# Feuermagier/Beyond_Deep_Ensembles

Hardware: NVIDIA B200
Metric: svgd_posterior_update_algorithmic_GBps (higher is better)
Workload: dtype f32

## Files before the change

beyond_deep_ensembles_b200/csrc/common.cuh:

```cuda
#pragma once
#include <cuda.h>
#include <cuda_runtime.h>
#include <cstdint>
#include <cstddef>

#include "bde_b200.h"

namespace bde {

#define BDE_RETURN_IF_CUDA(expr)                       \
    do {                                               \
        cudaError_t _e = (expr);                       \
        if (_e != cudaSuccess) return static_cast<int>(_e); \
    } while (0)

#define BDE_CHECK_LAUNCH()                             \
    do {                                               \
        cudaError_t _e = cudaGetLastError();           \
        if (_e != cudaSuccess) return static_cast<int>(_e); \
    } while (0)

inline int sm_count_cached() {
    static int cached[64] = {0};
    int dev = 0;
    if (cudaGetDevice(&dev) != cudaSuccess || dev < 0 || dev >= 64) return 148;
    if (cached[dev] == 0) {
        int v = 0;
        if (cudaDeviceGetAttribute(&v, cudaDevAttrMultiProcessorCount, dev) != cudaSuccess || v <= 0) v = 148;
        cached[dev] = v;
    }
    return cached[dev];
}

struct Tuning {
    int pairdist_ctas_per_sm = 0;
    int apply_ctas_per_sm = 0;
    int ew_ctas_per_sm = 0;
    int apply_variant = 0;
    int pairdist_variant = 0;
    int ew_variant = 0;
    int apply_tile_sets = 0;
    int swag_batch = 0;
    int batch_splits = 0;
    int batch_prefetch = 0;
    int gram_pairing = 0;
    int gram_fold = 0;
    int gram_l2_promotion = 0;
    int ring_kb = 0;
    int gram_guard_x1000 = 0;
};
Tuning& tuning();

inline bool aligned16(const void* p) { return (reinterpret_cast<uintptr_t>(p) & 15u) == 0; }

typedef unsigned long long f32x2;

__device__ __forceinline__ f32x2 pack2(float lo, float hi) {
    f32x2 r;
    asm("mov.b64 %0, {%1, %2};" : "=l"(r) : "f"(lo), "f"(hi));
    return r;
}
__device__ __forceinline__ void unpack2(f32x2 v, float& lo, float& hi) {
    asm("mov.b64 {%0, %1}, %2;" : "=f"(lo), "=f"(hi) : "l"(v));
}
__device__ __forceinline__ f32x2 sub2(f32x2 a, f32x2 b) {
    f32x2 r;
    asm("sub.f32x2 %0, %1, %2;" : "=l"(r) : "l"(a), "l"(b));
    return r;
}
__device__ __forceinline__ f32x2 add2(f32x2 a, f32x2 b) {
    f32x2 r;
    asm("add.f32x2 %0, %1, %2;" : "=l"(r) : "l"(a), "l"(b));
    return r;
}
__device__ __forceinline__ f32x2 mul2_rn(f32x2 a, f32x2 b) {
    f32x2 r;
    asm("mul.rn.f32x2 %0, %1, %2;" : "=l"(r) : "l"(a), "l"(b));
    return r;
}
__device__ __forceinline__ f32x2 add2_rn(f32x2 a, f32x2 b) {
    f32x2 r;
    asm("add.rn.f32x2 %0, %1, %2;" : "=l"(r) : "l"(a), "l"(b));
    return r;
}
__device__ __forceinline__ f32x2 fma2(f32x2 a, f32x2 b, f32x2 c) {
    f32x2 r;
    asm("fma.rn.f32x2 %0, %1, %2, %3;" : "=l"(r) : "l"(a), "l"(b), "l"(c));
    return r;
}
__device__ __forceinline__ f32x2 fma2s(float s, f32x2 b, f32x2 c) { return fma2(pack2(s, s), b, c); }

struct __align__(16) V4 {
    f32x2 lo, hi;
};

__device__ __forceinline__ V4 ldg_stream_v4(const float* p) {
    V4 v;
    asm volatile("ld.global.nc.L1::no_allocate.v2.u64 {%0, %1}, [%2];" : "=l"(v.lo), "=l"(v.hi) : "l"(p));
    return v;
}
__device__ __forceinline__ V4 ldg_cached_v4(const float* p) {
    V4 v;
    asm volatile("ld.global.nc.v2.u64 {%0, %1}, [%2];" : "=l"(v.lo), "=l"(v.hi) : "l"(p));
    return v;
}
__device__ __forceinline__ void stg_stream_v4(float* p, V4 v) {
    asm volatile("st.global.L1::no_allocate.v2.u64 [%0], {%1, %2};" ::"l"(p), "l"(v.lo), "l"(v.hi) : "memory");
}
__device__ __forceinline__ float4 ldg_stream_f4(const float* p) {
    float4 v;
    asm volatile("ld.global.nc.L1::no_allocate.v4.f32 {%0, %1, %2, %3}, [%4];"
                 : "=f"(v.x), "=f"(v.y), "=f"(v.z), "=f"(v.w)
                 : "l"(p));
    return v;
}
__device__ __forceinline__ float4 ld_f4(const float* p) {
    float4 v;
    asm volatile("ld.global.L1::no_allocate.v4.f32 {%0, %1, %2, %3}, [%4];"
                 : "=f"(v.x), "=f"(v.y), "=f"(v.z), "=f"(v.w)
                 : "l"(p));
    return v;
}
__device__ __forceinline__ void stg_stream_f4(float* p, float4 v) {
    asm volatile("st.global.L1::no_allocate.v4.f32 [%0], {%1, %2, %3, %4};" ::"l"(p), "f"(v.x), "f"(v.y),
                 "f"(v.z), "f"(v.w)
                 : "memory");
}

__device__ __forceinline__ uint32_t smem_u32(const void* p) { return static_cast<uint32_t>(__cvta_generic_to_shared(p)); }

__device__ __forceinline__ void mbar_init(uint64_t* bar, uint32_t count) {
    asm volatile("mbarrier.init.shared::cta.b64 [%0], %1;" ::"r"(smem_u32(bar)), "r"(count) : "memory");
}
__device__ __forceinline__ void mbar_fence_init() { asm volatile("fence.mbarrier_init.release.cluster;" ::: "memory"); }
__device__ __forceinline__ void mbar_arrive_expect_tx(uint64_t* bar, uint32_t bytes) {
    asm volatile("mbarrier.arrive.expect_tx.shared::cta.b64 _, [%0], %1;" ::"r"(smem_u32(bar)), "r"(bytes) : "memory");
}
__device__ __forceinline__ void mbar_arrive(uint64_t* bar) {
    asm volatile("mbarrier.arrive.shared::cta.b64 _, [%0];" ::"r"(smem_u32(bar)) : "memory");
}
__device__ __forceinline__ void mbar_wait(uint64_t* bar, uint32_t parity) {
    asm volatile(
        "{\n"
        ".reg .pred P1;\n"
        "LAB_WAIT:\n"
        "mbarrier.try_wait.parity.shared::cta.b64 P1, [%0], %1;\n"
        "@P1 bra DONE;\n"
        "bra LAB_WAIT;\n"
        "DONE:\n"
        "}" ::"r"(smem_u32(bar)),
        "r"(parity)
        : "memory");
}
__device__ __forceinline__ void tma_load_1d(void* smem_dst, const void* gmem_src, uint32_t bytes, uint64_t* bar) {
    asm volatile("cp.async.bulk.shared::cluster.global.mbarrier::complete_tx::bytes [%0], [%1], %2, [%3];" ::"r"(
                     smem_u32(smem_dst)),
                 "l"(gmem_src), "r"(bytes), "r"(smem_u32(bar))
                 : "memory");
}
__device__ __forceinline__ bool mbar_test(uint64_t* bar, uint32_t parity) {
    uint32_t ok;
    asm volatile(
        "{\n.reg .pred P1;\n"
        "mbarrier.test_wait.parity.shared::cta.b64 P1, [%1], %2;\n"
        "selp.u32 %0, 1, 0, P1;\n}"
        : "=r"(ok)
        : "r"(smem_u32(bar)), "r"(parity)
        : "memory");
    return ok != 0;
}
__device__ __forceinline__ void tma_load_2d(void* smem_dst, const CUtensorMap* map, int c0, int c1, uint64_t* bar) {
    asm volatile(
        "cp.async.bulk.tensor.2d.shared::cluster.global.tile.mbarrier::complete_tx::bytes [%0], [%1, {%2, %3}], [%4];" ::"r"(
            smem_u32(smem_dst)),
        "l"(reinterpret_cast<uint64_t>(map)), "r"(c0), "r"(c1), "r"(smem_u32(bar))
        : "memory");
}
__device__ __forceinline__ void tma_prefetch_map(const CUtensorMap* map) {
    asm volatile("prefetch.tensormap [%0];" ::"l"(reinterpret_cast<uint64_t>(map)) : "memory");
}
int encode_rows_tensor_map(CUtensorMap* map, const float* M, int rows, int64_t cols, int64_t ld, int box_cols,
                           int l2_promotion = 0);
constexpr int kTmaBoxCols = 256;

__device__ __forceinline__ V4 lds_v4(const float* p) {
    V4 v;
    asm volatile("ld.shared.v2.u64 {%0, %1}, [%2];" : "=l"(v.lo), "=l"(v.hi) : "r"(smem_u32(p)));
    return v;
}

__device__ __forceinline__ void griddep_launch() { asm volatile("griddepcontrol.launch_dependents;" ::: "memory"); }
__device__ __forceinline__ void griddep_wait() { asm volatile("griddepcontrol.wait;" ::: "memory"); }
bool take_chain_hint(cudaStream_t st);
bool& pdl_for_this_apply();

__device__ __forceinline__ float warp_sum(float v) {
#pragma unroll
    for (int o = 16; o > 0; o >>= 1) v += __shfl_xor_sync(0xffffffffu, v, o);
    return v;
}
__device__ __forceinline__ double warp_sum(double v) {
#pragma unroll
    for (int o = 16; o > 0; o >>= 1) v += __shfl_xor_sync(0xffffffffu, v, o);
    return v;
}

constexpr int kPeerMaxRanks = 16;
constexpr int kPeerMaxVals = 512;
struct PeerBuf {
    unsigned long long epoch;
    unsigned long long timeouts;
    unsigned long long wait_ns_sum;
    unsigned long long wait_ns_max;
    unsigned long long waits;
    unsigned long long pad[11];
    unsigned long long flags[2][kPeerMaxRanks][4];
    double slots[2][kPeerMaxRanks][kPeerMaxVals];
};
struct WsHeader {
    unsigned int ticket;
    int peer_world;
    int peer_rank;
    int redo;
    PeerBuf* peer[kPeerMaxRanks];
    unsigned long long timeout_ns;
    unsigned long long* host_status;
    int peer_failed;
};
constexpr size_t kWsHeaderBytes = 256;
static_assert(sizeof(WsHeader) <= kWsHeaderBytes, "workspace header");
constexpr unsigned long long kPeerTimeoutNs = 120ull * 1000 * 1000 * 1000;

__device__ __forceinline__ void st_relaxed_sys_f64(double* p, double v) {
    asm volatile("st.relaxed.sys.global.f64 [%0], %1;" ::"l"(p), "d"(v) : "memory");
}
__device__ __forceinline__ double ld_relaxed_sys_f64(const double* p) {
    double v;
    asm volatile("ld.relaxed.sys.global.f64 %0, [%1];" : "=d"(v) : "l"(p) : "memory");
    return v;
}
__device__ __forceinline__ void st_release_sys_u64(unsigned long long* p, unsigned long long v) {
    asm volatile("st.release.sys.global.u64 [%0], %1;" ::"l"(p), "l"(v) : "memory");
}
__device__ __forceinline__ unsigned long long ld_acquire_sys_u64(const unsigned long long* p) {
    unsigned long long v;
    asm volatile("ld.acquire.sys.global.u64 %0, [%1];" : "=l"(v) : "l"(p) : "memory");
    return v;
}
__device__ __forceinline__ unsigned long long globaltimer_ns() {
    unsigned long long t;
    asm volatile("mov.u64 %0, %globaltimer;" : "=l"(t));
    return t;
}

#ifdef BDE_TAIL_TIMING
#define BDE_TS_SLOT(ws_, i) (reinterpret_cast<unsigned long long*>(reinterpret_cast<char*>(ws_) + 192) + (i))
#define BDE_TS(ws_, i)                                                                       \
    do {                                                                                     \
        if (threadIdx.x == 0 && threadIdx.y == 0) *BDE_TS_SLOT(ws_, i) = globaltimer_ns();   \
    } while (0)
#define BDE_TS_MAX(ws_, i)                                                                             \
    do {                                                                                               \
        if (threadIdx.x == 0 && threadIdx.y == 0) atomicMax(BDE_TS_SLOT(ws_, i), globaltimer_ns());    \
    } while (0)
#else
#define BDE_TS(ws_, i) do { } while (0)
#define BDE_TS_MAX(ws_, i) do { } while (0)
#endif

__device__ __forceinline__ void peer_allreduce_fp64(WsHeader* h, double* total, int count) {
    const int world = h->peer_world;
    if (world <= 1) return;
    const int rank = h->peer_rank;
    const int tid = threadIdx.x + threadIdx.y * blockDim.x;
    const int nthreads = blockDim.x * blockDim.y;
    const double poison = __longlong_as_double(0x7ff8000000000000LL);
    if (h->peer_failed) {
        for (int k = tid; k < count; k += nthreads) total[k] = poison;
        __syncthreads();
        return;
    }
    PeerBuf* me = h->peer[rank];
    __shared__ unsigned long long s_epoch;
    __shared__ unsigned long long s_wait_ns;
    __shared__ int s_timed_out;
    if (tid == 0) {
        s_epoch = *reinterpret_cast<volatile unsigned long long*>(&me->epoch) + 1ull;
        s_timed_out = 0;
        s_wait_ns = 0ull;
    }
    __syncthreads();
    const unsigned long long epoch = s_epoch;
    const unsigned long long limit = h->timeout_ns ? h->timeout_ns : kPeerTimeoutNs;
    const int b = static_cast<int>(epoch & 1ull);
    for (int idx = tid; idx < world * count; idx += nthreads) {
        const int r = idx / count, k = idx - r * count;
        st_relaxed_sys_f64(&h->peer[r]->slots[b][rank][k], total[k]);
    }
    __threadfence_system();
    __syncthreads();
    if (tid < world) {
        st_release_sys_u64(&h->peer[tid]->flags[b][rank][0], epoch);
        const unsigned long long t0 = globaltimer_ns();
        while (ld_acquire_sys_u64(&me->flags[b][tid][0]) < epoch) {
            if (globaltimer_ns() - t0 > limit) {
                s_timed_out = 1;
                break;
            }
        }
        atomicMax(&s_wait_ns, globaltimer_ns() - t0);
    }
    __syncthreads();
    const bool bad = s_timed_out != 0;
    for (int k = tid; k < count; k += nthreads) {
        double s = 0.0;
        for (int r = 0; r < world; ++r) s += ld_relaxed_sys_f64(&me->slots[b][r][k]);
        total[k] = bad ? poison : s;
    }
    if (tid == 0) {
        *reinterpret_cast<volatile unsigned long long*>(&me->epoch) = epoch;
        me->wait_ns_sum += s_wait_ns;
        if (s_wait_ns > me->wait_ns_max) me->wait_ns_max = s_wait_ns;
        me->waits += 1ull;
        if (bad) {
            const unsigned long long nbad = me->timeouts + 1ull;
            *reinterpret_cast<volatile unsigned long long*>(&me->timeouts) = nbad;
            h->peer_failed = 1;
            if (h->host_status) {
                *reinterpret_cast<volatile unsigned long long*>(h->host_status) = nbad;
                __threadfence_system();
            }
        }
    }
    __syncthreads();
}
// ... 177 lines not shown
```

beyond_deep_ensembles_b200/csrc/svgd_gram.cu:

```cuda
#include "svgd_gram.cuh"

#include <cudaTypedefs.h>

namespace bde {

int encode_rows_tensor_map(CUtensorMap* map, const float* X, int n, int64_t D, int64_t ld, int box_cols, int l2_promotion) {
    static PFN_cuTensorMapEncodeTiled_v12000 encode = nullptr;
    if (!encode) {
        void* fn = nullptr;
        cudaDriverEntryPointQueryResult qres;
        BDE_RETURN_IF_CUDA(cudaGetDriverEntryPoint("cuTensorMapEncodeTiled", &fn, cudaEnableDefault, &qres));
        if (qres != cudaDriverEntryPointSuccess || !fn) return BDE_ERR_INVALID_ARG;
        encode = reinterpret_cast<PFN_cuTensorMapEncodeTiled_v12000>(fn);
    }
    if (!aligned16(X) || (ld % 4) != 0 || D < 1 || D > 0x7fffffffLL || n < 1 || n > 256 || box_cols > 256) return BDE_ERR_INVALID_ARG;
    const cuuint64_t dims[2] = {static_cast<cuuint64_t>(D), static_cast<cuuint64_t>(n)};
    const cuuint64_t strides[1] = {static_cast<cuuint64_t>(ld) * sizeof(float)};
    const cuuint32_t box[2] = {static_cast<cuuint32_t>(box_cols), static_cast<cuuint32_t>(n)};
    const cuuint32_t estr[2] = {1, 1};
    const CUtensorMapL2promotion promo = l2_promotion == 1 ? CU_TENSOR_MAP_L2_PROMOTION_L2_64B
                                         : l2_promotion == 2 ? CU_TENSOR_MAP_L2_PROMOTION_L2_128B
                                         : l2_promotion == 3 ? CU_TENSOR_MAP_L2_PROMOTION_L2_256B
                                                             : CU_TENSOR_MAP_L2_PROMOTION_NONE;
    const CUresult r = encode(map, CU_TENSOR_MAP_DATA_TYPE_FLOAT32, 2, const_cast<float*>(X), dims, strides, box, estr,
                              CU_TENSOR_MAP_INTERLEAVE_NONE, CU_TENSOR_MAP_SWIZZLE_NONE, promo,
                              CU_TENSOR_MAP_FLOAT_OOB_FILL_NONE);
    return r == CUDA_SUCCESS ? BDE_OK : BDE_ERR_INVALID_ARG;
}

template int launch_pairgram<16>(const float*, int64_t, int64_t, double*, void*, int, const BandwidthParams&, cudaStream_t);
template int launch_pairgram<20>(const float*, int64_t, int64_t, double*, void*, int, const BandwidthParams&, cudaStream_t);

}
```

beyond_deep_ensembles_b200/csrc/svgd_kernels.cuh:

```cuda
#pragma once
#include "common.cuh"
#include "svgd_internal.h"

namespace bde {

constexpr int kPairTarget = 48;
constexpr int kFlushIters = 128;
constexpr int kMaxCtasPairdist = 148 * 8 * 2;

__host__ __device__ constexpr int pair_count(int n) { return n * (n - 1) / 2; }
__host__ __device__ __forceinline__ constexpr int pair_index(int i, int j, int n) {
    return i * (2 * n - i - 1) / 2 + (j - i - 1);
}
__host__ __device__ constexpr int pair_row(int p, int n) {
    int i = 0;
    while (p >= n - 1 - i) {
        p -= n - 1 - i;
        ++i;
    }
    return i;
}
__host__ __device__ constexpr int pair_groups_contig(int n) {
    return pair_count(n) <= kPairTarget ? 1 : (pair_count(n) + kPairTarget - 1) / kPairTarget;
}
// ... 221 lines not shown
    __shared__ double s_h;
    int npad = 1;
    while (npad < nn) npad <<= 1;

    for (int e = tid; e < npad; e += nthreads) {
        double v = __longlong_as_double(0x7ff0000000000000LL);
        if (e < nn) {
            const double r = sqrt(dist[e]);
            v = r * r;
            sd[e] = v;
        }
        s_key[e] = v;
        s_ord[e] = e;
    }
    __syncthreads();
    for (int k = 2; k <= npad; k <<= 1) {
        for (int j = k >> 1; j > 0; j >>= 1) {
            for (int t = tid; t < (npad >> 1); t += nthreads) {
                const int i = ((t & ~(j - 1)) << 1) | (t & (j - 1));
                const int l = i | j;
                const bool up = (i & k) == 0;
                const double a = s_key[i], b = s_key[l];
                const int ia = s_ord[i], ib = s_ord[l];
                const bool gt = (a > b) || (a == b && ia > ib);
                if (gt == up) {
                    s_key[i] = b;
                    s_key[l] = a;
                    s_ord[i] = ib;
                    s_ord[l] = ia;
                }
            }
            const int j_next = j > 1 ? (j >> 1) : k;
            if (j <= 32 && j_next <= 32 && !(k == npad && j == 1))
                __syncwarp();
            else
                __syncthreads();
        }
    }
    const int pos_lo = (nn - 1) / 2;
    const int pos_hi = nn / 2;
    if (tid < 2) {
        const int pos = tid == 0 ? pos_lo : pos_hi;
        const int e = s_ord[pos];
        const int i = e / n, j = e - i * n;
        s_sel[tid] = s_key[pos];
        s_idx[tid] = i <= j ? e : j * n + i;
    }
    __syncthreads();
    if (tid == 0) {
        const double a = s_sel[0], b = s_sel[1];
        const double w = 0.5 * (nn - 1) - pos_lo;
        const double med = (w < 0.5) ? a + w * (b - a) : b - (b - a) * (1.0 - w);
        double h = sqrt(0.5 * med / log(static_cast<double>(n) + 1.0)) + 1e-8;
        if (bp.h_override > 0.0) h = bp.h_override;
        s_h = h;
        if (bp.info) {
            bp.info[0] = h;
            bp.info[1] = med;
            bp.info[2] = a;
            bp.info[3] = b;
        }
        if (bp.sel) {
            bp.sel[0] = s_idx[0];
            bp.sel[1] = s_idx[1];
        }
    }
    __syncthreads();
    const double h = s_h;
    const double inv2h2 = 1.0 / (2.0 * h * h);
    for (int e = tid; e < nn; e += nthreads) sk[e] = exp(-sd[e] * inv2h2);
    __syncthreads();
    const double c = bp.kernel_grad_scale / (bp.dataset_size * h * h);
    const double half_l2 = 0.5 * bp.l2_reg;
    for (int e = tid; e < nn; e += nthreads) {
        const int i = e / n, j = e - i * n;
        const double kij = sk[e];
        double a;
        if (i != j) {
            a = (half_l2 + c) * kij;
        } else {
            double off = 0.0;
            for (int m = 0; m < n; ++m)
                if (m != i) off += sk[i * n + m];
            a = half_l2 * kij - c * off;
        }
        bp.K[e] = static_cast<float>(kij);
        bp.A[e] = static_cast<float>(a);
    }
}

template <int MAXPAD>
__device__ __forceinline__ void bandwidth_device(const double* dist, int n, const BandwidthParams& bp, double* sd, double* sk) {
    __shared__ double s_key[MAXPAD];
    __shared__ int s_ord[MAXPAD];
    bandwidth_sorted(dist, n, bp, sd, sk, s_key, s_ord);
}


template <int N>
__global__ void __launch_bounds__(pairdist_tpb(N) * pair_groups(N))
svgd_pairdist_kernel(const float* __restrict__ X, int64_t D, int64_t ld, double* __restrict__ dist, int accumulate,
                     void* ws, int fuse_bandwidth, BandwidthParams bp, int only_if_redo) {
    if (only_if_redo && reinterpret_cast<const WsHeader*>(ws)->redo == 0) return;
    constexpr int P = pair_count(N);
    constexpr int PG = pairs_per_group(N);
    constexpr int NG = pair_groups(N);
    constexpr int TPB = pairdist_tpb(N);
    constexpr int WPG = TPB / 32;
    __shared__ double wacc[NG * WPG][PG];
    __shared__ double cta_vals[P];
    __shared__ double total[P];
    __shared__ double sd[N * N];
    __shared__ double sk[N * N];

    const int g = threadIdx.y;
    const int warp_in_group = threadIdx.x >> 5;
    const int tid = threadIdx.x + threadIdx.y * TPB;
    for (int k = tid; k < NG * WPG * PG; k += TPB * NG) (&wacc[0][0])[k] = 0.0;
    __syncthreads();

    group_dispatch<N, 0>(g, X, D, ld, wacc[g * WPG + warp_in_group]);
    __syncthreads();
    griddep_launch();

    for (int p = tid; p < P; p += TPB * NG) {
        const int i = pair_row(p, N), j = p - pair_index(i, i + 1, N) + i + 1;
        const int grp = pair_group_of(i, j, N), k = pair_slot_of(i, j, N);
        double s = 0.0;
#pragma unroll
        for (int w = 0; w < WPG; ++w) s += wacc[grp * WPG + w][k];
        cta_vals[p] = s;
    }
    __syncthreads();

    if (!grid_reduce_fp64(cta_vals, P, ws, total)) return;

    for (int e = tid; e < N * N; e += TPB * NG) {
        const int i = e / N, j = e - i * N;
        double v = 0.0;
        if (i != j) v = total[i < j ? pair_index(i, j, N) : pair_index(j, i, N)];
        if (accumulate) v += dist[e];
        dist[e] = v;
    }
    if (fuse_bandwidth && !peer_exchange_failed(ws)) {
        __syncthreads();
        bandwidth_device<pow2_ceil(N * N)>(dist, N, bp, sd, sk);
    }
}

__host__ __device__ constexpr int pd_tile_cols(int n) {
    return pair_groups(n) == 1 ? 1024 : (pair_groups(n) == 2 ? 512 : (pair_groups(n) <= 4 ? 256 : 128));
}
__host__ __device__ constexpr int pd_stage_bytes(int n) { return n * pd_tile_cols(n) * 4; }
__host__ __device__ constexpr int pd_stages(int n) {
    return (200 * 1024) / pd_stage_bytes(n) > 8 ? 8 : (200 * 1024) / pd_stage_bytes(n);
}
__host__ __device__ constexpr int pd_consumers(int n) { return pair_groups(n) * pd_tile_cols(n) / 4; }
constexpr int kFlushTiles = 64;

template <int N, int G>
__device__ __forceinline__ void pairdist_tma_consumer(const float* __restrict__ X, int64_t D, int64_t ld,
                                                      const float* __restrict__ tiles, uint64_t* full_bar,
                                                      uint64_t* empty_bar, double* __restrict__ wacc, int qi) {
    constexpr int PG = pairs_per_group(N);
    constexpr int TC = pd_tile_cols(N);
    constexpr int STAGES = pd_stages(N);
    f32x2 acc[PG > 0 ? PG : 1];
#pragma unroll
    for (int k = 0; k < PG; ++k) acc[k] = 0ull;
    const int lane = threadIdx.x & 31;
    const int64_t d4 = D & ~static_cast<int64_t>(3);
    const int64_t ntiles = (d4 + TC - 1) / TC;
    int it = 0;
    int64_t t = blockIdx.x;
    bool more = true;
    while (more) {
        for (int f = 0; f < kFlushTiles && t < ntiles; ++f, t += gridDim.x, ++it) {
            const int s = it % STAGES;
            const uint32_t use = static_cast<uint32_t>(it / STAGES);
            const int64_t col0 = t * TC;
            const int64_t w = (d4 - col0 < TC) ? d4 - col0 : TC;
            mbar_wait(&full_bar[s], use & 1u);
            const float* sx = tiles + static_cast<size_t>(s) * N * TC + 4 * qi;
            if constexpr (pair_blocked(N)) {
                const bool in = 4 * qi < w;
                pair_accumulate_blocked<N, G>(
                    [&](int r) {
                        V4 z;
                        z.lo = z.hi = 0ull;
                        return in ? lds_v4(sx + r * TC) : z;
                    },
                    [&] {
                        __syncwarp();
                        if (lane == 0) mbar_arrive(&empty_bar[s]);
                    },
                    acc);
            } else {
                V4 v[N];
                if (4 * qi < w) {
#pragma unroll
                    for (int i = 0; i < N; ++i) v[i] = lds_v4(sx + i * TC);
                } else {
#pragma unroll
                    for (int i = 0; i < N; ++i) v[i].lo = v[i].hi = 0ull;
                }
                __syncwarp();
                if (lane == 0) mbar_arrive(&empty_bar[s]);
                pair_accumulate<N, G>(v, acc);
            }
        }
        more = t < ntiles;
        if (!more && blockIdx.x == 0 && (D & 3)) {
            const int64_t c = d4 + qi;
            const bool in = qi < (D & 3);
            if constexpr (pair_blocked(N)) {
                pair_accumulate_blocked<N, G>(
                    [&](int r) {
                        V4 z;
                        z.lo = in ? pack2(__ldg(X + r * ld + c), 0.0f) : 0ull;
                        z.hi = 0ull;
                        return z;
                    },
                    [] {}, acc);
            } else {
                V4 v[N];
#pragma unroll
                for (int i = 0; i < N; ++i) {
                    v[i].lo = in ? pack2(__ldg(X + i * ld + c), 0.0f) : 0ull;
                    v[i].hi = 0ull;
                }
                pair_accumulate<N, G>(v, acc);
            }
        }
        flush_pairs<PG>(acc, wacc, lane);
    }
}

template <int N, int G>
__device__ __forceinline__ void pairdist_tma_dispatch(int g, const float* X, int64_t D, int64_t ld, const float* tiles,
                                                      uint64_t* full_bar, uint64_t* empty_bar, double* wacc, int qi) {
    if (g == G) {
        pairdist_tma_consumer<N, G>(X, D, ld, tiles, full_bar, empty_bar, wacc, qi);
    } else {
        if constexpr (G + 1 < pair_groups(N)) pairdist_tma_dispatch<N, G + 1>(g, X, D, ld, tiles, full_bar, empty_bar, wacc, qi);
    }
}

template <int N>
__global__ void __launch_bounds__(pd_consumers(N) + 32, 1)
svgd_pairdist_tma_kernel(const float* __restrict__ X, int64_t D, int64_t ld, double* __restrict__ dist, int accumulate,
                         void* ws, int fuse_bandwidth, BandwidthParams bp, int only_if_redo) {
    if (only_if_redo && reinterpret_cast<const WsHeader*>(ws)->redo == 0) return;
    constexpr int P = pair_count(N);
    constexpr int PG = pairs_per_group(N);
    constexpr int NG = pair_groups(N);
    constexpr int TC = pd_tile_cols(N);
    constexpr int QT = TC / 4;
    constexpr int STAGES = pd_stages(N);
    constexpr int kPdConsumers = pd_consumers(N);
    constexpr int CWARPS = kPdConsumers / 32;
    static_assert(QT % 32 == 0 && kPdConsumers <= 992, "consumer layout");
    extern __shared__ __align__(128) unsigned char smem_raw[];
    float* tiles = reinterpret_cast<float*>(smem_raw);
    __shared__ double wacc[CWARPS][PG];
    __shared__ double cta_vals[P];
    __shared__ double total[P];
    __shared__ double sd[N * N];
    __shared__ double sk[N * N];
    __shared__ __align__(8) uint64_t full_bar[STAGES];
    __shared__ __align__(8) uint64_t empty_bar[STAGES];

    const int tid = threadIdx.x;
    const int nthreads = kPdConsumers + 32;
    if (blockIdx.x == 0) BDE_TS(ws, 0);
    for (int k = tid; k < CWARPS * PG; k += nthreads) (&wacc[0][0])[k] = 0.0;
    if (tid == 0) {
#pragma unroll
        for (int s = 0; s < STAGES; ++s) {
            mbar_init(&full_bar[s], 1);
            mbar_init(&empty_bar[s], CWARPS);
        }
        mbar_fence_init();
    }
    __syncthreads();

    if (tid >= kPdConsumers) {
        if (tid == kPdConsumers) {
            const int64_t d4 = D & ~static_cast<int64_t>(3);
            const int64_t ntiles = (d4 + TC - 1) / TC;
            int it = 0;
            for (int64_t t = blockIdx.x; t < ntiles; t += gridDim.x, ++it) {
                const int s = it % STAGES;
                const uint32_t use = static_cast<uint32_t>(it / STAGES);
                mbar_wait(&empty_bar[s], (use & 1u) ^ 1u);
                const int64_t col0 = t * TC;
                const int64_t w = (d4 - col0 < TC) ? d4 - col0 : TC;
                const uint32_t row_bytes = static_cast<uint32_t>(w) * 4u;
                mbar_arrive_expect_tx(&full_bar[s], N * row_bytes);
                float* sx = tiles + static_cast<size_t>(s) * N * TC;
#pragma unroll
                for (int r = 0; r < N; ++r) tma_load_1d(sx + r * TC, X + r * ld + col0, row_bytes, &full_bar[s]);
            }
        }
    } else {
        const int wid = tid >> 5;
        const int g = wid % NG, qi = (wid / NG) * 32 + (tid & 31);
        pairdist_tma_dispatch<N, 0>(g, X, D, ld, tiles, full_bar, empty_bar, wacc[wid], qi);
    }
    __syncthreads();
    BDE_TS_MAX(ws, 1);
    griddep_launch();

    for (int p = tid; p < P; p += nthreads) {
        const int i = pair_row(p, N), j = p - pair_index(i, i + 1, N) + i + 1;
        const int grp = pair_group_of(i, j, N), k = pair_slot_of(i, j, N);
        double sacc = 0.0;
        for (int wv = grp; wv < CWARPS; wv += NG) sacc += wacc[wv][k];
        cta_vals[p] = sacc;
    }
    __syncthreads();
    if (!grid_reduce_fp64(cta_vals, P, ws, total)) return;
    for (int e = tid; e < N * N; e += nthreads) {
        const int i = e / N, j = e - i * N;
        double v = 0.0;
        if (i != j) v = total[i < j ? pair_index(i, j, N) : pair_index(j, i, N)];
        if (accumulate) v += dist[e];
        dist[e] = v;
    }
    BDE_TS(ws, 4);
    if (fuse_bandwidth && !peer_exchange_failed(ws)) {
        __syncthreads();
        bandwidth_device<pow2_ceil(N * N)>(dist, N, bp, sd, sk);
    }
    __syncthreads();
    BDE_TS(ws, 5);
#ifdef BDE_TAIL_TIMING
    if (fuse_bandwidth && !peer_exchange_failed(ws)) {
        __syncthreads();
        bandwidth_device<pow2_ceil(N * N)>(dist, N, bp, sd, sk);
    }
    __syncthreads();
    BDE_TS(ws, 6);
#endif
}

__host__ __device__ constexpr bool apply_rolled(int n) { return n > 16; }
__host__ __device__ constexpr bool apply_rolled(int n, int opt) { return n > 16 || (n == 16 && opt != kOptNone); }
__host__ __device__ constexpr int apply_row_chunk(int n) { return n <= 12 ? n : (n <= 16 ? 8 : 4); }

#ifndef BDE_APPLY_J_UNROLL
#define BDE_APPLY_J_UNROLL 5
#endif
template <int N, bool ROLLED = apply_rolled(N)>
__device__ __forceinline__ void apply_row(f32x2 (&acc)[N][2], const V4& g, const V4& x, const float* __restrict__ kt,
                                          const float* __restrict__ at) {
    if constexpr (N % 4 == 0 && ROLLED) {
#pragma unroll
        for (int c = 0; c < N / 4; ++c) {
            const float4 k4 = *reinterpret_cast<const float4*>(kt + 4 * c);
            const float4 a4 = *reinterpret_cast<const float4*>(at + 4 * c);
            const float kk[4] = {k4.x, k4.y, k4.z, k4.w};
            const float aa[4] = {a4.x, a4.y, a4.z, a4.w};
#pragma unroll
            for (int u = 0; u < 4; ++u) {
                const int i = 4 * c + u;
                acc[i][0] = fma2s(kk[u], g.lo, acc[i][0]);
                acc[i][1] = fma2s(kk[u], g.hi, acc[i][1]);
                acc[i][0] = fma2s(aa[u], x.lo, acc[i][0]);
                acc[i][1] = fma2s(aa[u], x.hi, acc[i][1]);
            }
        }
    } else {
#pragma unroll
        for (int i = 0; i < N; ++i) {
            const float kij = kt[i];
            const float aij = at[i];
            acc[i][0] = fma2s(kij, g.lo, acc[i][0]);
            acc[i][1] = fma2s(kij, g.hi, acc[i][1]);
            acc[i][0] = fma2s(aij, x.lo, acc[i][0]);
            acc[i][1] = fma2s(aij, x.hi, acc[i][1]);
        }
    }
}

__device__ __forceinline__ f32x2 mul2s(float s, f32x2 b) {
    f32x2 r;
    const f32x2 a = pack2(s, s);
    asm("mul.f32x2 %0, %1, %2;" : "=l"(r) : "l"(a), "l"(b));
    return r;
}
__device__ __forceinline__ V4 ld_coherent_v4(const float* p) {
    V4 v;
    asm volatile("ld.global.v2.u64 {%0, %1}, [%2];" : "=l"(v.lo), "=l"(v.hi) : "l"(p));
    return v;
}

__device__ __forceinline__ void sgd_update2(const BaseOptParams& o, bool clone_buf, f32x2 g, f32x2& x, f32x2& b) {
    if (o.weight_decay != 0.0f) g = fma2s(o.weight_decay, x, g);
    if (o.momentum != 0.0f) {
        if (clone_buf)
            b = g;
        else
            b = fma2s(o.one_minus_dampening, g, mul2s(o.momentum, b));
        g = o.nesterov ? fma2s(o.momentum, b, g) : b;
    }
    x = fma2s(-o.lr, g, x);
}

__device__ __forceinline__ float adam_update1(const BaseOptParams& o, int i, float g, float x, float& m, float& v) {
    if (o.weight_decay != 0.0f) {
        if (o.decoupled_wd)
            x = x * o.decay_factor;
        else
            g = fmaf(o.weight_decay, x, g);
    }
    m = fmaf(o.one_minus_beta1, g - m, m);
    v = fmaf(o.one_minus_beta2 * g, g, o.beta2 * v);
    const float denom = fmaf(sqrt_approx(v), o.inv_bc2_sqrt[i], o.eps);
    float r;
    asm("rcp.approx.ftz.f32 %0, %1;" : "=f"(r) : "f"(denom));
    return fmaf(-o.step_size[i] * m, r, x);
}
__device__ __forceinline__ void adam_update2(const BaseOptParams& o, int i, f32x2 g, f32x2& x, f32x2& m, f32x2& v) {
    if (o.weight_decay != 0.0f) {
        if (o.decoupled_wd)
            x = mul2s(o.decay_factor, x);
        else
            g = fma2s(o.weight_decay, x, g);
    }
    m = fma2s(o.one_minus_beta1, sub2(g, m), m);
    v = fma2(mul2s(o.one_minus_beta2, g), g, mul2s(o.beta2, v));
    float v0, v1, r0, r1;
    unpack2(v, v0, v1);
    const f32x2 denom = fma2s(o.inv_bc2_sqrt[i], pack2(sqrt_approx(v0), sqrt_approx(v1)), pack2(o.eps, o.eps));
    unpack2(denom, v0, v1);
    asm("rcp.approx.ftz.f32 %0, %1;" : "=f"(r0) : "f"(v0));
    asm("rcp.approx.ftz.f32 %0, %1;" : "=f"(r1) : "f"(v1));
    x = fma2(mul2s(-o.step_size[i], m), pack2(r0, r1), x);
}

template <int OPT>
__device__ __forceinline__ void opt_update_quad(const BaseOptParams& o, int i, f32x2 g_lo, f32x2 g_hi, V4& x, V4& s0, V4& s1) {
    if constexpr (OPT == kOptSgd) {
        const bool clone_buf = (i == 0) && !o.buf_initialized;
        sgd_update2(o, clone_buf, g_lo, x.lo, s0.lo);
        sgd_update2(o, clone_buf, g_hi, x.hi, s0.hi);
    } else if constexpr (OPT == kOptAdam) {
        adam_update2(o, i, g_lo, x.lo, s0.lo, s1.lo);
        adam_update2(o, i, g_hi, x.hi, s0.hi, s1.hi);
    }
}
__host__ __device__ constexpr int opt_state_rows(int opt) { return opt == kOptAdam ? 2 : (opt == kOptSgd ? 1 : 0); }

template <int OPT>
// ... 251 lines not shown
    if (is_producer) {
        if (tid == CONSUMERS) {
            int s = 0;
            uint32_t use = 0;
            for (int64_t t = blockIdx.x; t < ntiles; t += gridDim.x, s = (s + 1 == nst) ? 0 : s + 1, use += (s == 0)) {
                mbar_wait(&empty_bar[s], (use & 1u) ^ 1u);
                const int64_t col0 = t * TC;
                const int64_t w = (d4 - col0 < TC) ? d4 - col0 : TC;
                const uint32_t row_bytes = static_cast<uint32_t>(w) * 4u;
                const uint32_t nstate = (has_s0 ? 1u : 0u) + (OPT == kOptAdam ? 1u : 0u);
                mbar_arrive_expect_tx(&full_bar[s], 2u * N * TC * 4u + nstate * row_bytes);
                float* sx = tiles + static_cast<size_t>(s) * ROWS * TC;
                float* sg = sx + N * TC;
#pragma unroll
                for (int b = 0; b < NB; ++b) {
                    tma_load_2d(sx + b * N * BW, &mapX, static_cast<int>(col0) + b * BW, 0, &full_bar[s]);
                    tma_load_2d(sg + b * N * BW, &mapG, static_cast<int>(col0) + b * BW, 0, &full_bar[s]);
                }
                if constexpr (OPT != kOptNone) {
                    if (has_s0) tma_load_1d(sg + N * TC, o.state0 + col0, row_bytes, &full_bar[s]);
                    if (OPT == kOptAdam) tma_load_1d(sg + (N + 1) * TC, o.state1 + col0, row_bytes, &full_bar[s]);
                }
            }
        }
        griddep_wait();
    } else {
        griddep_wait();
        for (int e = tid; e < N * NP; e += CONSUMERS) {
            const int j = e / NP, i = e - j * NP;
            sKT[j][i] = (i < N) ? K[i * N + j] : 0.0f;
            sAT[j][i] = (i < N) ? A[i * N + j] : 0.0f;
        }
        asm volatile("bar.sync 1, %0;" ::"n"(CONSUMERS) : "memory");
        const int lane = tid & 31;
        const int set = tid / QT, q = tid - set * QT;
        f32x2 pacc[PN];
#pragma unroll
        for (int k = 0; k < PN; ++k) pacc[k] = 0ull;
        int it = set;
        int s = set;
        uint32_t use = 0;
        for (int64_t t = blockIdx.x + static_cast<int64_t>(set) * gridDim.x; t < ntiles;
             t += static_cast<int64_t>(TS) * gridDim.x, it += TS, s += TS, use += (s >= nst), s -= (s >= nst) ? nst : 0) {
            const int64_t col0 = t * TC;
            const int64_t w = (d4 - col0 < TC) ? d4 - col0 : TC;
            const bool active = 4 * q < w;
            if constexpr (TS > 1) {
                if (use > 0) mbar_wait(&empty_bar[s], (use - 1u) & 1u);
            }
            mbar_wait(&full_bar[s], use & 1u);
            const float* stage = tiles + static_cast<size_t>(s) * ROWS * TC;
            const float* sx = stage + (q / (BW / 4)) * (N * BW) + 4 * (q % (BW / 4));
            const float* sg = sx + N * TC;
            const float* sst = stage + 2 * N * TC + 4 * q;
            f32x2 acc[N][2];
#pragma unroll
            for (int i = 0; i < N; ++i) acc[i][0] = acc[i][1] = 0ull;
            if (active) {
                if constexpr (kApplyRolled) {
#pragma unroll(kApplyJUnroll)
                    for (int j = 0; j < N; ++j) apply_row<N, true>(acc, lds_v4(sg + j * BW), lds_v4(sx + j * BW), sKT[j], sAT[j]);
                } else {
#pragma unroll
                    for (int j = 0; j < N; ++j) apply_row<N>(acc, lds_v4(sg + j * BW), lds_v4(sx + j * BW), sKT[j], sAT[j]);
                }
            }
            if constexpr (OPT == kOptNone) {
                __syncwarp();
                if (lane == 0) mbar_arrive(&empty_bar[s]);
                if (active) {
                    float* op = out + col0 + 4 * q;
#pragma unroll
                    for (int i = 0; i < N; ++i) {
                        V4 v;
                        v.lo = acc[i][0];
                        v.hi = acc[i][1];
                        stg_stream_v4(op + i * ldo, v);
                    }
                }
            } else {
                V4 s0, s1;
                s0.lo = s0.hi = s1.lo = s1.hi = 0ull;
                V4 xn[NEXT ? N : 1];
                if constexpr (NEXT) {
#pragma unroll
                    for (int i = 0; i < N; ++i) xn[i].lo = xn[i].hi = 0ull;
                }
                if (active) {
                    float* xw = const_cast<float*>(X) + col0 + 4 * q;
                    if (has_s0) s0 = lds_v4(sst);
                    if (OPT == kOptAdam) s1 = lds_v4(sst + TC);
                    if (o.out_last) {
                        V4 v;
                        v.lo = acc[N - 1][0];
                        v.hi = acc[N - 1][1];
                        stg_stream_v4(o.out_last + col0 + 4 * q, v);
                    }
#pragma unroll
                    for (int i = 0; i < N; ++i) {
                        V4 x = lds_v4(sx + i * BW);
                        opt_update_quad<OPT>(o, i, acc[i][0], acc[i][1], x, s0, s1);
                        stg_stream_v4(xw + i * ldx, x);
                        if constexpr (NEXT) xn[i] = x;
                    }
                }
                __syncwarp();
                if (lane == 0) mbar_arrive(&empty_bar[s]);
                if (active) {
                    if (OPT == kOptAdam || o.momentum != 0.0f) stg_stream_v4(o.state0 + col0 + 4 * q, s0);
                    if (OPT == kOptAdam) stg_stream_v4(o.state1 + col0 + 4 * q, s1);
                }
                if constexpr (NEXT) {
                    pair_accumulate<N, 0>(xn, pacc);
                    if (((it / TS) % kFlushTiles) == kFlushTiles - 1) flush_pairs<PN>(pacc, wacc[tid >> 5], lane);
                }
            }
        }
        if constexpr (NEXT) {
            V4 xt[N];
#pragma unroll
            for (int i = 0; i < N; ++i) xt[i].lo = xt[i].hi = 0ull;
            if (blockIdx.x == 0 && tid < (D & 3)) {
                float xnew[N];
                apply_tail_column<N, OPT>(X, G, out, sKT, sAT, d4 + tid, ldx, ldg, ldo, o, xnew);
#pragma unroll
                for (int i = 0; i < N; ++i) xt[i].lo = pack2(xnew[i], 0.0f);
            }
            pair_accumulate<N, 0>(xt, pacc);
            flush_pairs<PN>(pacc, wacc[tid >> 5], lane);
        } else {
            if (blockIdx.x == 0 && tid < (D & 3)) apply_tail_column<N, OPT>(X, G, out, sKT, sAT, d4 + tid, ldx, ldg, ldo, o);
        }
    }
    if constexpr (NEXT) next_dist_epilogue<N, CWARPS>(wacc, nd);
}

template <int N>
int launch_pairdist(const float* X, int64_t D, int64_t ld, double* dist, int accumulate, void* ws, int fuse,
                    const BandwidthParams& bp, cudaStream_t st, int only_if_redo) {
    constexpr int TPB = pairdist_tpb(N);
    constexpr int NG = pair_groups(N);
    {
        constexpr int TC = pd_tile_cols(N);
        const int64_t ntiles = ((D & ~static_cast<int64_t>(3)) + TC - 1) / TC;
        int variant = tuning().pairdist_variant;
        if (variant == 0 || variant > 2) variant = (ntiles >= 2 * static_cast<int64_t>(sm_count_cached())) ? 2 : 1;
        if (variant == 2) {
            constexpr int smem = pd_stages(N) * pd_stage_bytes(N);
            static bool configured = false;
            if (!configured) {
                BDE_RETURN_IF_CUDA(cudaFuncSetAttribute(svgd_pairdist_tma_kernel<N>, cudaFuncAttributeMaxDynamicSharedMemorySize, smem));
                configured = true;
            }
            int64_t grid = sm_count_cached();
            if (grid > ntiles) grid = ntiles;
            if (grid < 1) grid = 1;
            svgd_pairdist_tma_kernel<N><<<static_cast<unsigned>(grid), pd_consumers(N) + 32, smem, st>>>(X, D, ld, dist, accumulate,
                                                                                                 ws, fuse, bp, only_if_redo);
            BDE_CHECK_LAUNCH();
            return BDE_OK;
        }
    }
    static int ctas_per_sm = 0;
    if (ctas_per_sm == 0) {
        int v = 0;
        BDE_RETURN_IF_CUDA(cudaOccupancyMaxActiveBlocksPerMultiprocessor(&v, svgd_pairdist_kernel<N>, TPB * NG, 0));
        ctas_per_sm = v > 0 ? v : 1;
    }
    const int64_t nquads = D >> 2;
    int64_t want = (nquads + TPB - 1) / TPB;
    int per_sm = ctas_per_sm;
    if (tuning().pairdist_ctas_per_sm > 0 && tuning().pairdist_ctas_per_sm < per_sm) per_sm = tuning().pairdist_ctas_per_sm;
    int64_t cap = static_cast<int64_t>(sm_count_cached()) * per_sm;
    if (tuning().pairdist_ctas_per_sm == 0 && want <= 16 * static_cast<int64_t>(sm_count_cached())) cap = sm_count_cached();
    if (cap > kMaxCtasPairdist) cap = kMaxCtasPairdist;
    if (want > cap) want = cap;
    if (want < 1) want = 1;
    svgd_pairdist_kernel<N><<<dim3(static_cast<unsigned>(want)), dim3(TPB, NG), 0, st>>>(X, D, ld, dist, accumulate, ws,
                                                                                      fuse, bp, only_if_redo);
    BDE_CHECK_LAUNCH();
    return BDE_OK;
}

template <int N, int OPT, bool NEXT, int TS, int TC>
int launch_apply_tma(const float* X, const float* G, float* out, const float* K, const float* A, int64_t D, int64_t ldx,
                     int64_t ldg, int64_t ldo, const BaseOptParams& o, cudaStream_t st, const NextDistParams& nd) {
    constexpr int smem = apply_stages(N, OPT, TC) * apply_stage_bytes(N, OPT, TC);
    static_assert(apply_stages(N, OPT, TC) >= 2, "ring too shallow");
    const int64_t d4 = D & ~static_cast<int64_t>(3);
    const int64_t ntiles = (d4 + TC - 1) / TC;
    static bool configured = false;
    if (!configured) {
        BDE_RETURN_IF_CUDA(cudaFuncSetAttribute(svgd_apply_tma_kernel<N, OPT, NEXT, TS, TC>, cudaFuncAttributeMaxDynamicSharedMemorySize, smem));
        configured = true;
    }
    CUtensorMap mapX, mapG;
    int rc = encode_rows_tensor_map(&mapX, X, N, d4, ldx, kTmaBoxCols);
    if (rc == BDE_OK) rc = encode_rows_tensor_map(&mapG, G, N, d4, ldg, kTmaBoxCols);
    if (rc != BDE_OK) return rc;
    int nst = apply_stages(N, OPT, TC);
    int ring_kb = tuning().ring_kb;
    if (ring_kb == 0 && OPT == kOptNone && !NEXT && N <= 12) ring_kb = 128;
    if (ring_kb > 0) {
        const int want = ring_kb * 1024 / apply_stage_bytes(N, OPT, TC);
        if (want < nst) nst = want > TS + 1 ? want : TS + 1;
    }
    int64_t grid = sm_count_cached();
    if (grid > ntiles) grid = ntiles;
    if (grid < 1) grid = 1;
    cudaLaunchConfig_t cfg = {};
    cfg.gridDim = dim3(static_cast<unsigned>(grid));
    cfg.blockDim = dim3(TS * (TC / 4) + 32);
    cfg.dynamicSmemBytes = smem;
    cfg.stream = st;
    cudaLaunchAttribute attr[1];
    attr[0].id = cudaLaunchAttributeProgrammaticStreamSerialization;
    attr[0].val.programmaticStreamSerializationAllowed = 1;
    cfg.attrs = attr;
    cfg.numAttrs = pdl_for_this_apply() ? 1 : 0;
    pdl_for_this_apply() = false;
    BDE_RETURN_IF_CUDA(cudaLaunchKernelEx(&cfg, svgd_apply_tma_kernel<N, OPT, NEXT, TS, TC>, mapX, mapG, X, G, out, K, A, D, ldx,
                                          ldg, ldo, o, nd, nst));
    return BDE_OK;
}

template <int N, int OPT, bool NEXT = false>
int launch_apply_opt(const float* X, const float* G, float* out, const float* K, const float* A, int64_t D, int64_t ldx,
                     int64_t ldg, int64_t ldo, const BaseOptParams& o, cudaStream_t st,
                     const NextDistParams& nd = NextDistParams{}) {
    const int64_t nquads = D >> 2;
    constexpr int TC = apply_tile_cols(N, OPT, NEXT);
    constexpr int TS0 = apply_default_tile_sets(N, OPT, NEXT);
    const int64_t d4 = D & ~static_cast<int64_t>(3);
    const int64_t ntiles = (d4 + TC - 1) / TC;
    int variant = tuning().apply_variant;
    if (variant == 0) {
        variant = (ntiles >= 2 * TS0 * static_cast<int64_t>(sm_count_cached()) || (!NEXT && d4 >= 65536)) ? 2 : 1;
    }
    if (d4 == 0 || d4 > 0x7fffffffLL) variant = 1;
    if (variant == 2) {
        constexpr int TS_ALT = !apply_small_tiles(N, OPT, NEXT) ? 3 : (N > 12 ? 7 - TS0 : 1);
        constexpr int TC_ALT = N > 12 ? 256 : 768 - TC;
        if (tuning().apply_tile_sets == TS_ALT) return launch_apply_tma<N, OPT, NEXT, TS_ALT, TC_ALT>(X, G, out, K, A, D, ldx, ldg, ldo, o, st, nd);
        if constexpr (!NEXT && OPT == kOptNone && N <= 12 && apply_small_tiles(N, OPT, NEXT)) {
            if (tuning().apply_tile_sets == 0 && static_cast<int64_t>(N) * ldx > kApplySmallTileMaxElems)
                return launch_apply_tma<N, OPT, NEXT, TS_ALT, TC_ALT>(X, G, out, K, A, D, ldx, ldg, ldo, o, st, nd);
        }
        return launch_apply_tma<N, OPT, NEXT, TS0, TC>(X, G, out, K, A, D, ldx, ldg, ldo, o, st, nd);
    }
    static int ctas_per_sm = 0;
    if (ctas_per_sm == 0) {
        int v = 0;
        BDE_RETURN_IF_CUDA(cudaOccupancyMaxActiveBlocksPerMultiprocessor(&v, svgd_apply_kernel<N, OPT, NEXT>, 128, 0));
        ctas_per_sm = v > 0 ? v : 1;
    }
    int64_t want = (nquads + 127) / 128;
    const int per_sm = tuning().apply_ctas_per_sm > 0 ? tuning().apply_ctas_per_sm : ctas_per_sm;
    int64_t cap = static_cast<int64_t>(sm_count_cached()) * per_sm;
    if (NEXT && tuning().apply_ctas_per_sm == 0 && want <= 16 * static_cast<int64_t>(sm_count_cached())) cap = sm_count_cached();
    if (NEXT && cap > kMaxCtasPairdist) cap = kMaxCtasPairdist;
    if (want > cap) want = cap;
    if (want < 1) want = 1;
    svgd_apply_kernel<N, OPT, NEXT><<<static_cast<unsigned>(want), 128, 0, st>>>(X, G, out, K, A, D, ldx, ldg, ldo, o, nd);
    BDE_CHECK_LAUNCH();
    return BDE_OK;
}

template <int N>
int launch_apply(const float* X, const float* G, float* out, const float* K, const float* A, int64_t D, int64_t ldx,
                 int64_t ldg, int64_t ldo, cudaStream_t st) {
    return launch_apply_opt<N, kOptNone>(X, G, out, K, A, D, ldx, ldg, ldo, BaseOptParams{}, st);
}

template <int N>
int launch_apply_fused(float* X, const float* G, const float* K, const float* A, int64_t D, int64_t ldx, int64_t ldg,
                       const BaseOptParams& o, cudaStream_t st, const NextDistParams* next) {
    if constexpr (N <= kNextDistMaxParticles) {
        if (next) {
            if (o.kind == kOptSgd) return launch_apply_opt<N, kOptSgd, true>(X, G, nullptr, K, A, D, ldx, ldg, 0, o, st, *next);
            return launch_apply_opt<N, kOptAdam, true>(X, G, nullptr, K, A, D, ldx, ldg, 0, o, st, *next);
        }
    } else {
        if (next) return BDE_ERR_UNSUPPORTED_N;
    }
    if (o.kind == kOptSgd) return launch_apply_opt<N, kOptSgd>(X, G, nullptr, K, A, D, ldx, ldg, 0, o, st);
    return launch_apply_opt<N, kOptAdam>(X, G, nullptr, K, A, D, ldx, ldg, 0, o, st);
}

}
```

Baseline: 6545.

## Load pairdist tiles with one 3D TMA tensor copy instead of per-row bulk copies

The TMA pairdist producer now encodes a 3D tensor map (256-column chunks × chunks × rows) and issues a single tensor-tile copy per full stage, replacing N separate 1D bulk copies. Partial tail tiles still use the old per-row path. For the single-group case the shared-memory ring is also cut from 200 KB to 120 KB, which changes the stage count. The aim is lower issue overhead on the producer thread, at the cost of encoding a tensor map on the host every launch and possibly fewer pipeline stages.

New measurement: 6676, median of 6. 2.0% higher.

```diff
diff --git a/beyond_deep_ensembles_b200/csrc/common.cuh b/beyond_deep_ensembles_b200/csrc/common.cuh
--- a/beyond_deep_ensembles_b200/csrc/common.cuh
+++ b/beyond_deep_ensembles_b200/csrc/common.cuh
@@ -176,11 +176,19 @@
         "l"(reinterpret_cast<uint64_t>(map)), "r"(c0), "r"(c1), "r"(smem_u32(bar))
         : "memory");
 }
+__device__ __forceinline__ void tma_load_3d(void* smem_dst, const CUtensorMap* map, int c0, int c1, int c2, uint64_t* bar) {
+    asm volatile(
+        "cp.async.bulk.tensor.3d.shared::cluster.global.tile.mbarrier::complete_tx::bytes [%0], [%1, {%2, %3, %4}], [%5];" ::"r"(
+            smem_u32(smem_dst)),
+        "l"(reinterpret_cast<uint64_t>(map)), "r"(c0), "r"(c1), "r"(c2), "r"(smem_u32(bar))
+        : "memory");
+}
 __device__ __forceinline__ void tma_prefetch_map(const CUtensorMap* map) {
     asm volatile("prefetch.tensormap [%0];" ::"l"(reinterpret_cast<uint64_t>(map)) : "memory");
 }
 int encode_rows_tensor_map(CUtensorMap* map, const float* M, int rows, int64_t cols, int64_t ld, int box_cols,
                            int l2_promotion = 0);
+int encode_chunks_tensor_map(CUtensorMap* map, const float* M, int rows, int64_t chunks, int64_t ld, int box_chunks);
 constexpr int kTmaBoxCols = 256;
 
 __device__ __forceinline__ V4 lds_v4(const float* p) {
diff --git a/beyond_deep_ensembles_b200/csrc/svgd_gram.cu b/beyond_deep_ensembles_b200/csrc/svgd_gram.cu
--- a/beyond_deep_ensembles_b200/csrc/svgd_gram.cu
+++ b/beyond_deep_ensembles_b200/csrc/svgd_gram.cu
@@ -4,7 +4,7 @@
 
 namespace bde {
 
-int encode_rows_tensor_map(CUtensorMap* map, const float* X, int n, int64_t D, int64_t ld, int box_cols, int l2_promotion) {
+static int tensor_map_encoder(PFN_cuTensorMapEncodeTiled_v12000* out) {
     static PFN_cuTensorMapEncodeTiled_v12000 encode = nullptr;
     if (!encode) {
         void* fn = nullptr;
@@ -13,6 +13,13 @@
         if (qres != cudaDriverEntryPointSuccess || !fn) return BDE_ERR_INVALID_ARG;
         encode = reinterpret_cast<PFN_cuTensorMapEncodeTiled_v12000>(fn);
     }
+    *out = encode;
+    return BDE_OK;
+}
+
+int encode_rows_tensor_map(CUtensorMap* map, const float* X, int n, int64_t D, int64_t ld, int box_cols, int l2_promotion) {
+    PFN_cuTensorMapEncodeTiled_v12000 encode = nullptr;
+    if (const int rc = tensor_map_encoder(&encode); rc != BDE_OK) return rc;
     if (!aligned16(X) || (ld % 4) != 0 || D < 1 || D > 0x7fffffffLL || n < 1 || n > 256 || box_cols > 256) return BDE_ERR_INVALID_ARG;
     const cuuint64_t dims[2] = {static_cast<cuuint64_t>(D), static_cast<cuuint64_t>(n)};
     const cuuint64_t strides[1] = {static_cast<cuuint64_t>(ld) * sizeof(float)};
@@ -28,6 +35,23 @@
     return r == CUDA_SUCCESS ? BDE_OK : BDE_ERR_INVALID_ARG;
 }
 
+int encode_chunks_tensor_map(CUtensorMap* map, const float* X, int n, int64_t chunks, int64_t ld, int box_chunks) {
+    PFN_cuTensorMapEncodeTiled_v12000 encode = nullptr;
+    if (const int rc = tensor_map_encoder(&encode); rc != BDE_OK) return rc;
+    constexpr int64_t kChunk = kTmaBoxCols;
+    if (!aligned16(X) || (ld % 4) != 0 || chunks < 1 || kChunk * chunks > ld || n < 1 || n > 256 || box_chunks < 1 ||
+        box_chunks > 256)
+        return BDE_ERR_INVALID_ARG;
+    const cuuint64_t dims[3] = {static_cast<cuuint64_t>(kChunk), static_cast<cuuint64_t>(chunks), static_cast<cuuint64_t>(n)};
+    const cuuint64_t strides[2] = {static_cast<cuuint64_t>(kChunk) * sizeof(float), static_cast<cuuint64_t>(ld) * sizeof(float)};
+    const cuuint32_t box[3] = {static_cast<cuuint32_t>(kChunk), static_cast<cuuint32_t>(box_chunks), static_cast<cuuint32_t>(n)};
+    const cuuint32_t estr[3] = {1, 1, 1};
+    const CUresult r = encode(map, CU_TENSOR_MAP_DATA_TYPE_FLOAT32, 3, const_cast<float*>(X), dims, strides, box, estr,
+                              CU_TENSOR_MAP_INTERLEAVE_NONE, CU_TENSOR_MAP_SWIZZLE_NONE, CU_TENSOR_MAP_L2_PROMOTION_NONE,
+                              CU_TENSOR_MAP_FLOAT_OOB_FILL_NONE);
+    return r == CUDA_SUCCESS ? BDE_OK : BDE_ERR_INVALID_ARG;
+}
+
 template int launch_pairgram<16>(const float*, int64_t, int64_t, double*, void*, int, const BandwidthParams&, cudaStream_t);
 template int launch_pairgram<20>(const float*, int64_t, int64_t, double*, void*, int, const BandwidthParams&, cudaStream_t);
 
diff --git a/beyond_deep_ensembles_b200/csrc/svgd_kernels.cuh b/beyond_deep_ensembles_b200/csrc/svgd_kernels.cuh
--- a/beyond_deep_ensembles_b200/csrc/svgd_kernels.cuh
+++ b/beyond_deep_ensembles_b200/csrc/svgd_kernels.cuh
@@ -397,8 +397,10 @@
     return pair_groups(n) == 1 ? 1024 : (pair_groups(n) == 2 ? 512 : (pair_groups(n) <= 4 ? 256 : 128));
 }
 __host__ __device__ constexpr int pd_stage_bytes(int n) { return n * pd_tile_cols(n) * 4; }
+constexpr int kPdRingKbOneGroup = 120;
+__host__ __device__ constexpr int pd_ring_bytes(int n) { return (pair_groups(n) == 1 ? kPdRingKbOneGroup : 200) * 1024; }
 __host__ __device__ constexpr int pd_stages(int n) {
-    return (200 * 1024) / pd_stage_bytes(n) > 8 ? 8 : (200 * 1024) / pd_stage_bytes(n);
+    return pd_ring_bytes(n) / pd_stage_bytes(n) > 8 ? 8 : pd_ring_bytes(n) / pd_stage_bytes(n);
 }
 __host__ __device__ constexpr int pd_consumers(int n) { return pair_groups(n) * pd_tile_cols(n) / 4; }
 constexpr int kFlushTiles = 64;
@@ -493,8 +495,9 @@
 
 template <int N>
 __global__ void __launch_bounds__(pd_consumers(N) + 32, 1)
-svgd_pairdist_tma_kernel(const float* __restrict__ X, int64_t D, int64_t ld, double* __restrict__ dist, int accumulate,
-                         void* ws, int fuse_bandwidth, BandwidthParams bp, int only_if_redo) {
+svgd_pairdist_tma_kernel(const __grid_constant__ CUtensorMap mapX, const float* __restrict__ X, int64_t D, int64_t ld,
+                         double* __restrict__ dist, int accumulate, void* ws, int fuse_bandwidth, BandwidthParams bp,
+                         int only_if_redo) {
     if (only_if_redo && reinterpret_cast<const WsHeader*>(ws)->redo == 0) return;
     constexpr int P = pair_count(N);
     constexpr int PG = pairs_per_group(N);
@@ -505,6 +508,7 @@
     constexpr int kPdConsumers = pd_consumers(N);
     constexpr int CWARPS = kPdConsumers / 32;
     static_assert(QT % 32 == 0 && kPdConsumers <= 992, "consumer layout");
+    static_assert(TC % kTmaBoxCols == 0, "a tile is whole 256-column chunks of the tensor map");
     extern __shared__ __align__(128) unsigned char smem_raw[];
     float* tiles = reinterpret_cast<float*>(smem_raw);
     __shared__ double wacc[CWARPS][PG];
@@ -533,6 +537,7 @@
         if (tid == kPdConsumers) {
             const int64_t d4 = D & ~static_cast<int64_t>(3);
             const int64_t ntiles = (d4 + TC - 1) / TC;
+            if (d4 >= TC) tma_prefetch_map(&mapX);
             int it = 0;
             for (int64_t t = blockIdx.x; t < ntiles; t += gridDim.x, ++it) {
                 const int s = it % STAGES;
@@ -540,11 +545,16 @@
                 mbar_wait(&empty_bar[s], (use & 1u) ^ 1u);
                 const int64_t col0 = t * TC;
                 const int64_t w = (d4 - col0 < TC) ? d4 - col0 : TC;
-                const uint32_t row_bytes = static_cast<uint32_t>(w) * 4u;
-                mbar_arrive_expect_tx(&full_bar[s], N * row_bytes);
                 float* sx = tiles + static_cast<size_t>(s) * N * TC;
-#pragma unroll
-                for (int r = 0; r < N; ++r) tma_load_1d(sx + r * TC, X + r * ld + col0, row_bytes, &full_bar[s]);
+                if (w == TC) {
+                    mbar_arrive_expect_tx(&full_bar[s], N * TC * 4u);
+                    tma_load_3d(sx, &mapX, 0, static_cast<int>(col0 / kTmaBoxCols), 0, &full_bar[s]);
+                } else {
+                    const uint32_t row_bytes = static_cast<uint32_t>(w) * 4u;
+                    mbar_arrive_expect_tx(&full_bar[s], N * row_bytes);
+#pragma unroll
+                    for (int r = 0; r < N; ++r) tma_load_1d(sx + r * TC, X + r * ld + col0, row_bytes, &full_bar[s]);
+                }
             }
         }
     } else {
@@ -1102,11 +1112,17 @@
                 BDE_RETURN_IF_CUDA(cudaFuncSetAttribute(svgd_pairdist_tma_kernel<N>, cudaFuncAttributeMaxDynamicSharedMemorySize, smem));
                 configured = true;
             }
+            CUtensorMap mapX{};
+            const int64_t d4 = D & ~static_cast<int64_t>(3);
+            if (d4 >= TC) {
+                const int rc = encode_chunks_tensor_map(&mapX, X, N, d4 / kTmaBoxCols, ld, TC / kTmaBoxCols);
+                if (rc != BDE_OK) return rc;
+            }
             int64_t grid = sm_count_cached();
             if (grid > ntiles) grid = ntiles;
             if (grid < 1) grid = 1;
-            svgd_pairdist_tma_kernel<N><<<static_cast<unsigned>(grid), pd_consumers(N) + 32, smem, st>>>(X, D, ld, dist, accumulate,
-                                                                                                 ws, fuse, bp, only_if_redo);
+            svgd_pairdist_tma_kernel<N><<<static_cast<unsigned>(grid), pd_consumers(N) + 32, smem, st>>>(
+                mapX, X, D, ld, dist, accumulate, ws, fuse, bp, only_if_redo);
             BDE_CHECK_LAUNCH();
             return BDE_OK;
         }
```
